# wreuven/h264-scroll-encoder

Measured on AMD Instinct MI355X. Metric: composed frames/sec (1280x720, 360x360 dyn) at 1/2/4/8 GPU; bit-exact vs CPU, higher is better.
Workload: dtype u8; 1 GPU; BASELINE config 3: 256 concurrent 1280x720 streams + 360x360 synthetic dynamic rect (4x4 int transform + quant + CAVLC), composer_write_scroll_frame semantics; resolution=1280x720, streams_per_gpu=256, parallelism=static stream shard x1, no RCCL

## Files before the change

h264-scroll-encoder_amd/csrc/dyn_device.h:

```cpp
#ifndef SCROLL_DYN_DEVICE_H
#define SCROLL_DYN_DEVICE_H

#include "qparams.h"
#include "scroll_device.h"

namespace scroll {
namespace dyn {

constexpr int QP_DEFAULT = 26, QP_MIN = 22, QP_MAX = 51, LEVEL_MAX = 2063;
__host__ __device__ constexpr int mf_of(int r, int cls)
{
    constexpr int T[6][3] = {{13107, 5243, 8066}, {11916, 4660, 7490}, {10082, 4194, 6554},
                             {9362, 3647, 5825},  {8192, 3355, 5243},  {7282, 2893, 4559}};
    return T[r][cls];
}
__host__ __device__ constexpr QParams qparams(int qp)
{
    return QParams{mf_of(qp % 6, 0), mf_of(qp % 6, 1), mf_of(qp % 6, 2), 15 + qp / 6, (1 << (15 + qp / 6)) / 6};
}
__device__ __host__ inline QParams qparams_rt(int qp)
{
    const int r = qp % 6, b = 15 + qp / 6;
    const int m0 = r == 0 ? 13107 : r == 1 ? 11916 : r == 2 ? 10082 : r == 3 ? 9362 : r == 4 ? 8192 : 7282;
    const int m1 = r == 0 ? 5243 : r == 1 ? 4660 : r == 2 ? 4194 : r == 3 ? 3647 : r == 4 ? 3355 : 2893;
// ... 881 lines not shown
        const int p = top_bit(mm);
        mm &= ~(1u << p);
        const int run = pprev - p - 1;
        const uint32_t e = P.rb[(zl < 7 ? zl : 7) - 1][run];
        push(acc, an, e & 255u, e >> 8, cap);
        zl -= run;
        pprev = p;
    }
    if constexpr (LB) {
        if (cap.n == 0) {
            cap.lo = acc;
            cap.n = an;
            ok = true;
            return tc;
        }
    }
    if (an > 32u) cap.put((uint32_t)(acc >> 32), (int)(an - 32u));
    cap.put((uint32_t)acc, an > 32u ? 32 : (int)an);
    ok = cap.n <= 128;
    return tc;
}

constexpr int TZRB_N = 65536 + 32768;
__device__ __host__ inline uint32_t tzrb_entry(const Tabs &T, uint32_t nz, int maxc)
{
    const int tc = __builtin_popcount(nz);
    if (tc == 0) return 1u << 31;
    uint32_t acc = 0;
    int n = 0;
    const int hi = 31 - __builtin_clz(nz), tz = hi + 1 - tc;
    if (tc < maxc) {
        acc = T.tz_bits[tc - 1][tz];
        n = T.tz_len[tc - 1][tz];
    }
    int zl = tz, p = hi;
    uint32_t m = nz & ~(1u << hi);
    for (int k = 1; k < tc && zl > 0; ++k) {
        const int q = 31 - __builtin_clz(m);
        m &= ~(1u << q);
        const int run = p - q - 1, zi = (zl < 7 ? zl : 7) - 1;
        acc = (acc << T.rb_len[zi][run]) | T.rb_bits[zi][run];
        n += T.rb_len[zi][run];
        zl -= run;
        p = q;
    }
    return (n ? acc << (32 - n) : 0u) | (1u << (31 - n));
}

constexpr int LVT_V = 47, LVT_W = 96, LVT_C = 9, LVT_N = LVT_C * LVT_W, LVT_ROW = 4 * LVT_W;
__device__ __host__ constexpr uint32_t lvt_entry(int c, int v)
{
    if (v == 0 || v > LVT_V || v < -LVT_V) return 0u;
    const int sl = c >= 7 ? c - 7 : c, adj = c >= 7 ? 2 : 0;
    const int a = v < 0 ? -v : v;
    const int code = 2 * a - 2 + (v < 0 ? 1 : 0) - adj;
    if (code < 0) return 0u;
    const int lim = sl ? (15 << sl) : 30;
    const uint32_t mk = (1u << sl) - 1u;
    uint32_t fv = ((uint32_t)code & mk) | (mk + 1u), fl = (uint32_t)((code >> sl) + 1 + sl);
    if (code >= lim) {
        fv = (uint32_t)(4096 + code - lim);
        fl = 28u;
    } else if (sl == 0 && code >= 14) {
        fv = (uint32_t)(code + 2);
        fl = 19u;
    }
    const int s1 = sl == 0 ? 1 : sl;
    const int nx = s1 + ((a > (3 << (s1 - 1)) && s1 < 6) ? 1 : 0);
    return fv | fl << 13 | (uint32_t)(nx * LVT_ROW) << 18;
}
struct LvTab {
    uint32_t e[LVT_N];
};
constexpr LvTab make_lvt()
{
    LvTab T{};
    for (int c = 0; c < LVT_C; ++c)
        for (int i = 0; i < LVT_W; ++i) T.e[c * LVT_W + i] = lvt_entry(c, i - LVT_V - 1);
    return T;
}

template <class CAP>
__device__ __host__ inline int cavlc_body_t(CAP &cap, const int8_t *lb, uint32_t nz, uint32_t tzrb, int &t1o,
                                            bool &ok, const uint32_t *lvt)
{
    const int tc = __builtin_popcount(nz);
    const uint32_t g0 = (nz << 1) | 1u;
    const int c0 = __builtin_clz(g0);
    const uint32_t g1 = g0 & ~((0x80000000u >> c0) & ~1u);
    const int c1 = __builtin_clz(g1);
    const uint32_t g2 = g1 & ~((0x80000000u >> c1) & ~1u);
    const int c2 = __builtin_clz(g2);
    const uint32_t g3 = g2 & ~((0x80000000u >> c2) & ~1u);
    const int v0 = lb[30 - c0], v1 = lb[30 - c1], v2 = lb[30 - c2];
    const bool o0 = c0 < 31 && v0 * v0 == 1, o1 = o0 && c1 < 31 && v1 * v1 == 1;
    const bool o2 = o1 && c2 < 31 && v2 * v2 == 1;
    const int t1 = (int)o0 + (int)o1 + (int)o2;
    t1o = t1;
    ok = true;
    if (tc == 0) return 0;
    const uint32_t s3 = ((uint32_t)v0 >> 31) << 2 | ((uint32_t)v1 >> 31) << 1 | ((uint32_t)v2 >> 31);
    uint64_t acc = s3 >> (3 - t1);
    uint32_t an = (uint32_t)t1;
    uint32_t g = t1 == 0 ? g0 : (t1 == 1 ? g1 : (t1 == 2 ? g2 : g3));
    uint32_t m = g >> 1;
    auto push = [](uint64_t &ac, uint32_t &n, uint32_t v, uint32_t len, CAP &c) {
        uint32_t n2 = n + len;
        if (n2 > 64u) {
            if (n > 32u) c.put((uint32_t)(ac >> 32), (int)(n - 32u));
            c.put((uint32_t)ac, n > 32u ? 32 : (int)n);
            ac = 0;
            n2 = len;
        }
        ac = (ac << len) | v;
        n = n2;
    };
    uint32_t cls = (uint32_t)((((tc > 10 && t1 < 3) ? 1 : 0) + (t1 < 3 ? 7 : 0)) * LVT_ROW);
    auto entry = [lvt](uint32_t row, int v) -> uint32_t {
        return *reinterpret_cast<const uint32_t *>(reinterpret_cast<const char *>(lvt + LVT_V + 1) + ((int)row + 4 * v));
    };
    auto level_code = [&](int v, uint32_t row) -> uint32_t {
        if (v >= -LVT_V && v <= LVT_V) return entry(row, v);
        const int cl = (int)row / LVT_ROW;
        const int sl = cl >= 7 ? cl - 7 : cl, adj = cl >= 7 ? 2 : 0;
        const int a = v < 0 ? -v : v;
        const int code = 2 * a - 2 + (v < 0 ? 1 : 0) - adj;
        const int lim = sl ? (15 << sl) : 30;
        const uint32_t mk = (1u << sl) - 1u;
        uint32_t fv = ((uint32_t)code & mk) | (mk + 1u);
        uint32_t fl = (uint32_t)((code >> sl) + 1 + sl);
        const bool e15 = code >= lim, e14 = sl == 0 && code >= 14;
        fv = e15 ? (uint32_t)(4096 + code - lim) : (e14 ? (uint32_t)(code + 2) : fv);
        fl = e15 ? 28u : (e14 ? 19u : fl);
        const int s1 = sl == 0 ? 1 : sl;
        return fv | fl << 13 | (uint32_t)((s1 + ((a > (3 << (s1 - 1)) && s1 < 6) ? 1 : 0)) * LVT_ROW) << 18;
    };
    const uint32_t m0 = m, an0 = an;
    const uint64_t acc0 = acc;
    const uint32_t cls0 = cls;
    const CAP cap0 = cap;
    uint32_t big = 0;
    int cn = __builtin_clz(g);
    int vn = (int)lb[30 - cn];
    while (g > 1u) {
        const int v = vn;
        g &= ~(0x80000000u >> cn);
        cn = __builtin_clz(g);
        vn = (int)lb[30 - cn];
        const int vc = v < -LVT_V ? -LVT_V : (v > LVT_V ? LVT_V : v);
        big |= (uint32_t)(vc ^ v);
        const uint32_t e = entry(cls, vc);
        push(acc, an, e & 0x1fffu, (e >> 13) & 31u, cap);
        cls = e >> 18;
    }
    if (big) {
        m = m0;
        an = an0;
        acc = acc0;
        cls = cls0;
        cap = cap0;
        for (int k = t1; k < tc; ++k) {
            const int p = top_bit(m);
            m &= ~(1u << p);
            const uint32_t e = level_code((int)lb[p], cls);
            push(acc, an, e & 0x1fffu, (e >> 13) & 31u, cap);
            cls = e >> 18;
        }
    }
    const uint32_t tzl = 31u - (uint32_t)__builtin_ctz(tzrb);
    push(acc, an, (tzrb >> 1) >> (31u - tzl), tzl, cap);
    if (cap.n == 0) {
        cap.lo = acc;
        cap.n = an;
        return tc;
    }
    if (an > 32u) cap.put((uint32_t)(acc >> 32), (int)(an - 32u));
    cap.put((uint32_t)acc, an > 32u ? 32 : (int)an);
    ok = cap.n <= 128;
    return tc;
}

template <class CAP, class PT>
__device__ __host__ inline int cavlc_dc4(CAP &cap, const PT &P, const int c[4])
{
    const uint32_t nz = (c[0] != 0 ? 1u : 0u) | (c[1] != 0 ? 2u : 0u) | (c[2] != 0 ? 4u : 0u) |
                        (c[3] != 0 ? 8u : 0u);
// ... 109 lines not shown
```

h264-scroll-encoder_amd/csrc/dyn_kernels.hip:

```cpp
#include <hip/hip_runtime.h>

#include <stdint.h>
#include <mutex>

#include "dyn_device.h"
#include "dyn_engine.h"
#include "nal_ctx.h"
#include "stage_util.h"

using namespace scroll;
using namespace scroll::dyn;
using namespace scroll::stage;

namespace {

__constant__ Tabs g_tabs = SCROLL_DYN_TABS;
constexpr Tabs k_tabs = SCROLL_DYN_TABS;
__constant__ PTabs g_ptabs = make_ptabs(k_tabs);
__device__ uint32_t g_tzrb[TZRB_N];
struct QpPair {
    QParams l, c;
};
struct QpTab {
    QpPair q[QP_MAX + 1];
// ... 904 lines not shown
                     rowstage + nb * g.rs_frame_words + rs_runs_words(g, nA, gi), EPC_STATIC - 1, t, GW);
        wave_sync();
    }
    if (t == 0) rowstage[nb * g.rs_frame_words + rs_runs_words(g, nA, gi)] = L.ncand;
}


__device__ inline CapSink cap_of_msb(uint64_t a, uint64_t b, uint32_t n)
{
    if (n == 0u) return CapSink{0, 0, 0};
    const uint32_t sh = 128u - n;
    if (sh >= 64u) return CapSink{0, a >> (sh - 64u), n};
    if (sh == 0u) return CapSink{a, b, n};
    return CapSink{a >> sh, (b >> sh) | (a << (64u - sh)), n};
}

__device__ inline void put_piece(uint32_t *buf, uint32_t p0, uint32_t n, uint32_t pos, uint32_t tv, uint32_t tl,
                                 uint4 b, uint32_t bl)
{
    const uint32_t tw = tv & low_mask((int)tl);
    const uint32_t c0 = __builtin_amdgcn_alignbit(tw, b.x, tl), c1 = __builtin_amdgcn_alignbit(b.x, b.y, tl);
    const uint32_t c2 = __builtin_amdgcn_alignbit(b.y, b.z, tl), c3 = __builtin_amdgcn_alignbit(b.z, b.w, tl);
    const uint32_t c4 = __builtin_amdgcn_alignbit(b.w, 0u, tl);
    const uint32_t sh = pos & 31u;
    const uint32_t o[6] = {c0 >> sh, __builtin_amdgcn_alignbit(c0, c1, sh), __builtin_amdgcn_alignbit(c1, c2, sh),
                           __builtin_amdgcn_alignbit(c2, c3, sh), __builtin_amdgcn_alignbit(c3, c4, sh),
                           __builtin_amdgcn_alignbit(c4, 0u, sh)};
    const uint32_t nw = (sh + tl + bl + 31u) >> 5, w0 = (pos >> 5) - p0;
#pragma unroll
    for (uint32_t j = 0; j < 6; ++j)
        if (j < nw && w0 + j < n && o[j]) atomicOr(&buf[w0 + j], o[j]);
}

constexpr uint32_t ROW_PAD = 4;

__device__ inline void put_piece1(uint32_t *buf, uint32_t pos, uint32_t tv, uint32_t tl, uint4 b, uint32_t bl)
{
    const uint32_t tw = tv & low_mask((int)tl);
    const uint32_t c0 = __builtin_amdgcn_alignbit(tw, b.x, tl), c1 = __builtin_amdgcn_alignbit(b.x, b.y, tl);
    const uint32_t c2 = __builtin_amdgcn_alignbit(b.y, b.z, tl), c3 = __builtin_amdgcn_alignbit(b.z, b.w, tl);
    const uint32_t c4 = __builtin_amdgcn_alignbit(b.w, 0u, tl);
    const uint32_t sh = pos & 31u, nw = (sh + tl + bl + 31u) >> 5;
    uint32_t *d = buf + (pos >> 5);
    atomicOr(d, c0 >> sh);
    if (nw > 1u) atomicOr(d + 1, __builtin_amdgcn_alignbit(c0, c1, sh));
    if (nw > 2u) atomicOr(d + 2, __builtin_amdgcn_alignbit(c1, c2, sh));
    if (nw > 3u) {
        atomicOr(d + 3, __builtin_amdgcn_alignbit(c2, c3, sh));
        if (nw > 4u) {
            atomicOr(d + 4, __builtin_amdgcn_alignbit(c3, c4, sh));
            if (nw > 5u) atomicOr(d + 5, __builtin_amdgcn_alignbit(c4, 0u, sh));
        }
    }
}

constexpr int ROW_MAXT = 1024;
#ifndef SCROLL_ROW_WAVES
#define SCROLL_ROW_WAVES 8
#endif
#ifndef SCROLL_ROW_NP
#define SCROLL_ROW_NP 3
#endif
#ifndef SCROLL_ROW_NP_WIDE
#define SCROLL_ROW_NP_WIDE 4
#endif
#ifndef SCROLL_ROW_WIDE
#define SCROLL_ROW_WIDE 40
#endif
constexpr int ROW_NPMAX = 8;
#ifndef SCROLL_ROW_GB
#define SCROLL_ROW_GB 896
#endif
constexpr int ROW_GB = SCROLL_ROW_GB;

constexpr int ROW_PCD_N = (NPC + 3) & ~3;

struct RowFixed {
    RowTabs ptabs;
    uint32_t pcd[ROW_PCD_N];
    union {
        uint32_t buf[ROW_GB + 4];
        struct {
            uint32_t kc[2][SORT_KEYS];
            uint32_t kc_pad[32 - 2 * SORT_KEYS];
            uint32_t lvt[LVT_N];
        };
    };
    uint64_t hhi[12], hlo[12];
    uint32_t hlen[12];
    int32_t wo[8], wl[8], wv[8];
    int32_t head_over;
    uint32_t rt[32];
    uint32_t ncand;
    uint32_t spill;
};

static_assert(2 * SORT_KEYS <= 32 && 32 + LVT_N <= ROW_GB, "the sort counts and the level table share the bit window");
static_assert(ROW_PAD == 4, "RowFixed::buf holds ROW_PAD spare words");
static_assert(sizeof(RowFixed) <= 4992, "eight config-3 row workgroups per CU");

__host__ __device__ inline size_t row_lds_base(int w)
{
    return (size_t)16 * NPC * w + (size_t)4 * (w + 1) + (size_t)2 * (3 * NPC * w) + (size_t)10 * w + 16;
}
#ifndef SCROLL_ROW_GB_WIDE
#define SCROLL_ROW_GB_WIDE 1248
#endif
constexpr int ROW_GB_WIDE = SCROLL_ROW_GB_WIDE;
__host__ __device__ inline size_t row_wide_off(int w) { return (row_lds_base(w) + 15) & ~(size_t)15; }
__host__ __device__ inline bool row_wide_win(int w)
{
    return w > SCROLL_ROW_WIDE && row_wide_off(w) + 4 * (size_t)(ROW_GB_WIDE + ROW_PAD) + sizeof(RowFixed) <= 163840;
}
__host__ __device__ inline size_t row_lds_bytes(int w)
{
    return row_wide_win(w) ? row_wide_off(w) + 4 * (size_t)(ROW_GB_WIDE + ROW_PAD) : row_lds_base(w);
}

__host__ __device__ constexpr uint32_t pc_desc(int pc)
{
    if (pc == 16 || pc == 17) return 1u << 17;
    int da = 0, db = 0, e = 0;
    bool al = false, bt = false;
    if (pc < 16) {
        const int bx = pc & 3, by = pc >> 2;
        al = bx == 0;
        da = al ? 3 - NPC : -1;
        bt = by == 0;
        db = bt ? 0 : -4;
        e = bt ? pc : 0;
    } else {
        const int b = (pc - 18) & 3, bx = b & 1, by = b >> 1;
        al = bx == 0;
        da = al ? 1 - NPC : -1;
        bt = by == 0;
        db = bt ? 0 : -2;
        e = bt ? (pc < 22 ? pc - 14 : pc - 16) : 0;
    }
    return (uint32_t)(da + 32) | (al ? 1u : 0u) << 6 | (uint32_t)(db + 32) << 7 | (bt ? 1u : 0u) << 13 |
           (uint32_t)e << 14;
}

struct alignas(16) RowConst {
    RowTabs ptabs;
    uint32_t pcd[ROW_PCD_N];
    uint32_t lvt[LVT_N];
};
constexpr RowConst make_rowconst(const Tabs &T)
{
    RowConst C{};
    const PTabs P = make_ptabs(T);
    for (int i = 0; i < 4 * 68; ++i) C.ptabs.ct[i / 68][i % 68] = P.ct[i / 68][i % 68];
    for (int i = 0; i < 12; ++i) C.ptabs.tzdc[i / 4][i % 4] = P.tzdc[i / 4][i % 4];
    for (int i = 0; i < 7 * 16; ++i) C.ptabs.rb[i / 16][i % 16] = P.rb[i / 16][i % 16];
    for (int i = 0; i < NPC; ++i) C.pcd[i] = pc_desc(i);
    const LvTab V = make_lvt();
    for (int i = 0; i < LVT_N; ++i) C.lvt[i] = V.e[i];
    return C;
}
__constant__ RowConst g_rowconst = make_rowconst(k_tabs);
constexpr int ROWC_NV = (int)(sizeof(RowConst) / 16), ROWC_HEAD = (int)(offsetof(RowConst, lvt) / 16);
constexpr int ROWC_GAP = (int)((offsetof(RowFixed, lvt) - offsetof(RowConst, lvt)) / 16);
static_assert(offsetof(RowFixed, ptabs) == 0 && offsetof(RowFixed, pcd) == offsetof(RowConst, pcd) &&
                  offsetof(RowFixed, kc) == offsetof(RowConst, lvt) && offsetof(RowFixed, lvt) % 16 == 0 &&
                  sizeof(RowConst) % 16 == 0 && sizeof(RowConst) == 16 * ROWC_HEAD + 4 * LVT_N,
              "RowConst is RowFixed's head without the sort's words");
static_assert(offsetof(RowFixed, wl) == offsetof(RowFixed, wo) + 32 && offsetof(RowFixed, wv) == offsetof(RowFixed, wo) + 64 &&
                  offsetof(PlanPending, wl) == offsetof(PlanPending, wo) + 32 &&
                  offsetof(PlanPending, wv) == offsetof(PlanPending, wo) + 64,
              "the waypoint table copies as 24 words");

struct EpfLds {
    uint32_t *goff, *gb, *gw, *cw, *cbase, *lst, *cnt;
    uint32_t *ws;
};
__host__ __device__ inline int row_chroma0(int w) { return (16 * w + 63) & ~63; }
__host__ __device__ inline int row_vtasks(int w) { return row_chroma0(w) + 8 * w; }

__host__ __device__ inline int row_threads(int w)
{
    const int nt = row_vtasks(w), np = w > SCROLL_ROW_WIDE ? SCROLL_ROW_NP_WIDE : SCROLL_ROW_NP;
    const int a = (((nt + np - 1) / np) + 63) & ~63;
    const int b = (((nt + ROW_NPMAX - 1) / ROW_NPMAX) + 63) & ~63;
    const int t = a > b ? a : b;
    return t < ROW_MAXT ? t : ROW_MAXT;
}

struct BlkPix {
    uint32_t a[4], b[4], c;
};

__device__ inline __amdgpu_buffer_rsrc_t buf_rsrc(const void *p, uint32_t n)
{
    return __builtin_amdgcn_make_buffer_rsrc(const_cast<void *>(p), (short)0, (int)n, 0x00020000);
}

struct FetchOff {
    uint32_t s, b[4], c;
    int pb;
};

__device__ inline void fetch_luma(FetchOff &o, int v, int ry, const DynGeom &g, const uint32_t *rt)
{
    const int k = v >> 4, r = v & 15, bx = r & 3, by = r >> 2;
    o.s = (uint32_t)((16 * ry + 4 * by) * (16 * g.w) + 16 * k + 4 * bx);
    const uint32_t po = (uint32_t)(16 * (g.x0 + k) + 4 * bx);
#pragma unroll
    for (int i = 0; i < 4; ++i) o.b[i] = po + rt[4 * by + i];
    o.c = o.b[3];
}

__device__ inline void fetch_chroma(FetchOff &o, int e, int ry, const DynGeom &g, uint32_t csz, const uint32_t *ru,
                                    const uint32_t *rd)
{
    const int ndt = g.w * g.h, k = e >> 3, p = (e >> 2) & 1, r = e & 3, bx = r & 1, by = r >> 1;
    o.s = (uint32_t)(256 * ndt + (p ? 64 * ndt : 0) + (8 * ry + 4 * by) * (8 * g.w) + 8 * k + 4 * bx);
    const uint32_t co = (uint32_t)p * csz + (uint32_t)(8 * (g.x0 + k) + 4 * bx);
#pragma unroll
    for (int i = 0; i < 4; ++i) o.b[i] = co + (ru[4 * by + i] & ROW_OFF);
    o.c = co + (rd[4 * by + 3] & ROW_OFF);
}

__device__ inline void fetch_pass9(const FetchOff &o, uint32_t adv, uint32_t stride, __amdgpu_buffer_rsrc_t fs,
                                   __amdgpu_buffer_rsrc_t rb, BlkPix &px)
{
#pragma unroll
    for (int i = 0; i < 4; ++i) {
        px.a[i] = __builtin_amdgcn_raw_buffer_load_b32(fs, o.s, adv + (uint32_t)i * stride, 0);
        px.b[i] = __builtin_amdgcn_raw_buffer_load_b32(rb, o.b[i], adv, 0);
    }
    px.c = __builtin_amdgcn_raw_buffer_load_b32(rb, o.c, adv, 0);
}

__device__ inline uint32_t bilin4(uint32_t b, uint32_t c, uint32_t f)
{
    const uint32_t g = 8u - f;
    const uint32_t be = b & 0x00ff00ffu, bo = (b >> 8) & 0x00ff00ffu;
    const uint32_t ce = c & 0x00ff00ffu, co = (c >> 8) & 0x00ff00ffu;
    const uint32_t ve = __umul24(g, be) + __umul24(f, ce) + 0x00040004u;
    const uint32_t vo = __umul24(g, bo) + __umul24(f, co) + 0x00040004u;
    return ((ve >> 3) & 0x00ff00ffu) | (((vo >> 3) & 0x00ff00ffu) << 8);
}

static_assert(NPC == 26 && NPC * DYN_MAX_W < 18724, "div_npc's reciprocal (10083 / 2^18) is exact below 18724");
__device__ inline int div_npc(int i) { return (int)(__umul24((uint32_t)i, 10083u) >> 18); }

__device__ inline int row_slot(int task, int w)
{
    const int jj = task - 16 * w;
    const bool l = jj < 0;
    const int k = l ? task >> 4 : jj >> 3, pc = l ? task & 15 : 18 + (jj & 7);
    return (int)__umul24((uint32_t)k, (uint32_t)NPC) + pc;
}

struct RowArgs {
    DevStream *st;
    const NalDesc *nal;
    const PlanPending *pend;
    DynFrame *dfr;
    const uint32_t *rows;
    const uint8_t *src, *refs;
    const uint4 *heads;
    int32_t ld_nal, ld_fr;
    DynGeom g;
    unsigned long long *tcx;
    uint32_t epoch, pad0;
    uint32_t *rowstage, *gbits, *spill, *ctr;
    const uint16_t *meta;
    const uint2 *blo, *bhi;
    const uint4 *bwd;
    uint64_t *stamps;
};
static_assert(std::is_trivially_copyable<RowArgs>::value && std::is_standard_layout<RowArgs>::value,
              "RowArgs is copied into the kernel-argument segment as it is: offsetof = kernarg offset");
static_assert(offsetof(RowArgs, st) == 0 && alignof(RowArgs) == 8 && sizeof(RowArgs) % 8 == 0,
              "the only kernel parameter starts the kernel-argument segment");
static_assert(offsetof(RowArgs, tcx) % 16 == 0 && offsetof(RowArgs, epoch) == offsetof(RowArgs, tcx) + 8,
              "tcx and epoch: one 16-byte scalar load");
static_assert(offsetof(RowArgs, gbits) == offsetof(RowArgs, rowstage) + 8 &&
                  offsetof(RowArgs, ctr) == offsetof(RowArgs, rowstage) + 24,
              "phase 5's four pointers are adjacent");

typedef const char __attribute__((address_space(4))) *KargPtr;
__device__ inline KargPtr kargs_here()
{
    KargPtr p = (KargPtr)__builtin_amdgcn_kernarg_segment_ptr();
    asm volatile("" : "+s"(p));
    return p;
}
template <class T>
__device__ inline T karg_at(KargPtr p, size_t off)
{
    return *reinterpret_cast<const T __attribute__((address_space(4))) *>(p + off);
}
#define row_arg(K, F) karg_at<decltype(RowArgs::F)>(K, offsetof(RowArgs, F))

__device__ inline void row_copy_tabs(RowFixed &L, int s, size_t nb, int lane)
{
    constexpr int NK = (ROWC_NV + 63) / 64;
    const KargPtr K = kargs_here();
    const int32_t *pw = reinterpret_cast<const int32_t *>(reinterpret_cast<const char *>(row_arg(K, pend) + s) +
                                                          offsetof(PlanPending, wo));
    const uint4 *hv = row_arg(K, heads) + nb * DYN_HEAD_VECS;
    const uint4 *src = reinterpret_cast<const uint4 *>(&g_rowconst);
    const int l24 = min(lane, 23), l12 = min(lane, 11);
    uint4 v[NK];
#pragma unroll
    for (int k = 0; k < NK; ++k) v[k] = src[min(lane + 64 * k, ROWC_NV - 1)];
    const int32_t wp = pw[l24];
    const uint4 m = hv[l12];
    const uint32_t hl = reinterpret_cast<const uint32_t *>(hv + 12)[l12];
    uint4 *dst = reinterpret_cast<uint4 *>(&L);
#pragma unroll
    for (int k = 0; k < NK; ++k) {
        const int i = min(lane + 64 * k, ROWC_NV - 1);
        dst[i + (i >= ROWC_HEAD ? ROWC_GAP : 0)] = v[k];
    }
    reinterpret_cast<int32_t *>(reinterpret_cast<char *>(&L) + offsetof(RowFixed, wo))[l24] = wp;
    L.hhi[l12] = (uint64_t)m.x << 32 | m.y;
    L.hlo[l12] = (uint64_t)m.z << 32 | m.w;
    L.hlen[l12] = hl & 0x7fffffffu;
    const bool over = __builtin_amdgcn_ballot_w64(lane < 12 && (hl >> 31)) != 0;
    if (lane == 0) L.head_over = over;
}

template <bool GEN, bool DBG>
__global__ __launch_bounds__(ROW_MAXT) __attribute__((amdgpu_waves_per_eu(SCROLL_ROW_WAVES))) void k_dyn_row(const RowArgs a)
{
    __shared__ RowFixed L;
    extern __shared__ uint4 rdyn[];
    const DynGeom &g = a.g;
    uint64_t *const stamps = DBG ? a.stamps : nullptr;
    const uint64_t t_entry = stamps ? __builtin_amdgcn_s_memrealtime() : 0ull;
    const int r = blockIdx.x, t = threadIdx.x, T = blockDim.x, lane = t & 63, wave = t >> 6, nwv = T >> 6;
    int f = blockIdx.y, s = blockIdx.z;
    const int ld_fr = a.ld_fr;
    if (GEN) {
        const uint32_t *ctr = a.ctr;
        const uint32_t j = blockIdx.y, n = min(__builtin_amdgcn_readfirstlane(ctr[1]), g.gen_cap);
        if (j >= n) return;
        const uint32_t q = __builtin_amdgcn_readfirstlane(ctr[DYN_CTR_LIST + j]);
        s = (int)(q / (uint32_t)ld_fr);
        f = (int)(q - (uint32_t)s * (uint32_t)ld_fr);
    }
    const size_t nb = (size_t)s * ld_fr + f;
    constexpr bool general = GEN;
    constexpr int SR = DYN_STATIC_ROWS;
    uint64_t *stp = nullptr;
    if (DBG && stamps) stp = stamps + (((size_t)s * gridDim.y + f) * g.ngroups + (max(1, (g.y0 + SR - 1) / SR) + r)) * 8;
    if (stp && t == 0) stp[0] = t_entry;
    const Rect R{g.x0, g.y0, g.w, g.h};
    const int w = R.w, ndt = R.w * R.h, row = R.y0 + r, npc = NPC * w, ntask = 24 * w;
    const int nA = max(1, (R.y0 + SR - 1) / SR);
    const DevStream *S = a.st + s;
    const uint32_t *const rows = a.rows;
    const int mbw = g.pw / 16;
    const uint32_t ysz = (uint32_t)g.pw * (uint32_t)g.ph, csz = ysz / 4;
    const int L0 = row_chroma0(w), nl = 16 * w, ntv = L0 + 8 * w;
    const int np = (ntv + T - 1) / T;
    const int wv0 = 64 * __builtin_amdgcn_readfirstlane(wave);
    auto kind_of = [&](int q) -> int {
        const int v0 = q * T + wv0;
        return v0 < nl ? 0 : (v0 < ntv ? 1 : 2);
    };
    const __amdgpu_buffer_rsrc_t fs = buf_rsrc(a.src + (size_t)s * g.src_ld + (size_t)f * g.src_fr, (uint32_t)g.src_fr);
    const __amdgpu_buffer_rsrc_t rb = buf_rsrc(a.refs + (size_t)s * g.ref_ld, 3u * ysz);
    const DynFrame df = a.dfr[nb];
    FetchOff fo;
    fo.pb = -1;
    bool fo_chroma = false;
    BlkPix nx;
    if (!general) {
        const uint32_t *rtg = rows + nb * (size_t)(32 * g.h);
        const int k0 = kind_of(0);
        const int e = t & 31;
        const uint32_t rtv = rtg[e < 16 ? 16 * r + e : 16 * g.h + (e < 24 ? 8 * r + e - 16 : 8 * g.h + 8 * r + e - 24)];
        if (k0 == 0) {
            fetch_luma(fo, t, r, g, rtg + 16 * r);
            fo.pb = 0;
            fetch_pass9(fo, 0u, (uint32_t)(16 * w), fs, rb, nx);
            nx.c = 0u;
            L.rt[e] = rtv;
        } else if (k0 == 1) {
            fetch_chroma(fo, t - L0, r, g, csz, rtg + 16 * g.h + 8 * r, rtg + 24 * g.h + 8 * r);
            fo.pb = 0;
            fo_chroma = true;
            fetch_pass9(fo, 0u, (uint32_t)(8 * w), fs, rb, nx);
        }
    }
    if (df.nal < 0 || ((df.err & DF_GENERAL) != 0) != GEN) return;

    uint4 *lv = rdyn;
    uint32_t *moff = reinterpret_cast<uint32_t *>(lv + npc);
    uint16_t *mt = reinterpret_cast<uint16_t *>(moff + w + 1), *lo = mt + npc, *off16 = lo + npc;
    uint16_t *order = off16;
    uint8_t *ta = reinterpret_cast<uint8_t *>(off16 + npc), *cbpa = ta + 8 * w, *codea = cbpa + w;
    uint32_t *mbits = reinterpret_cast<uint32_t *>(ta);

    if (t == 0) L.ncand = 0;
    if (t < SORT_KEYS) L.kc[0][t] = 0u;
    if (general && wv0 == T - 64) row_copy_tabs(L, s, nb, lane);
    const int qpy = __builtin_amdgcn_readfirstlane((int)df.ep);
    const QParams ql = g_qptab.q[qpy].l, qc = g_qptab.q[qpy].c;
    const HeadSel HS = head_sel(S, a.nal[(size_t)s * a.ld_nal + df.nal]);
    if (!general)
        asm volatile(""
                     :
                     : "s"(HS.a_end), "s"(HS.mbw), "s"(ql.mf0), "s"(ql.mf1), "s"(ql.mf2), "s"(ql.qbits), "s"(ql.qf),
                       "s"(qc.mf0), "s"(qc.mf1), "s"(qc.mf2), "s"(qc.qbits), "s"(qc.qf));

    __syncthreads();
    if (!general) {
        static_assert(ROW_MAXT % 64 == 0, "row_threads gives whole waves: the per-pass step T is a multiple of 64");
        const uint32_t frc = __builtin_amdgcn_readfirstlane((L.rt[16] >> 28) & 7u);
        const int qL = nl > wv0 ? (nl - wv0 + T - 1) / T : 0;
        const int qC = ntv > wv0 ? (ntv - wv0 + T - 1) / T : 0;
        auto issue_l = [&](int q, BlkPix &px) {
            fetch_pass9(fo, (uint32_t)((q - fo.pb) * T), (uint32_t)(16 * w), fs, rb, px);
        };
        auto issue_c = [&](int q, BlkPix &px) {
            if (!fo_chroma) {
                fetch_chroma(fo, q * T + t - L0, r, g, csz, L.rt + 16, L.rt + 24);
                fo.pb = q;
                fo_chroma = true;
            }
            fetch_pass9(fo, (uint32_t)((q - fo.pb) * T), (uint32_t)(8 * w), fs, rb, px);
        };
        auto issue_any = [&](int q, BlkPix &px) {
            if (q < qL) issue_l(q, px);
            else issue_c(q, px);
        };
        const NzConst nzc = nz_const();
        auto put_rec = [&](int slot, const uint32_t pk[4]) {
            const uint4 p4 = make_uint4(pk[0], pk[1], pk[2], pk[3]);
            const uint32_t nz = nz_mask16_c(p4, nzc);
            const int n = __builtin_popcount(nz);
            lv[slot] = p4;
            mt[slot] = (uint16_t)nz;
            if (n) lo[slot] = (uint16_t)atomicAdd(&L.kc[0][SORT_KEYS - 1 - min(n, SORT_KEYS - 1)], 1u);
        };
        const LevelsBias bl = levels_bias(ql), bc = levels_bias(qc);
        auto code_l = [&](int q, const BlkPix &px) {
            const int v = q * T + t;
            uint32_t pk[4];
            int w0 = 0;
            levels_pk<true>(px.a, px.b, pk, w0, ql, bl.k1, bl.k0);
            if (v < nl) put_rec((int)__umul24((uint32_t)(v >> 4), (uint32_t)NPC) + (v & 15), pk);
        };
        auto code_c = [&](int q, const BlkPix &px) {
            const int e = q * T + t - L0;
            uint32_t pr[4], pk[4];
            int w0 = 0;
            if (frc == 4u) {
#pragma unroll
                for (int i = 0; i < 4; ++i) pr[i] = __builtin_amdgcn_lerp(px.b[i], i < 3 ? px.b[i + 1] : px.c, 0x01010101u);
            } else if (frc == 0u) {
#pragma unroll
                for (int i = 0; i < 4; ++i) pr[i] = px.b[i];
            } else {
#pragma unroll
                for (int i = 0; i < 4; ++i) pr[i] = bilin4(px.b[i], i < 3 ? px.b[i + 1] : px.c, frc);
            }
            levels_pk<false>(px.a, pr, pk, w0, qc, bc.k1, bc.k0);
            const bool ok = e < 8 * w;
            if (ok) put_rec((int)__umul24((uint32_t)(e >> 3), (uint32_t)NPC) + 18 + (e & 7), pk);
            if (ok) reinterpret_cast<int16_t *>(lv + (e >> 3) * NPC + 16 + ((e >> 2) & 1))[e & 3] = (int16_t)w0;
        };
        BlkPix A = nx, B;
        int q = 0;
        for (; q + 1 < qL; q += 2) {
            issue_l(q + 1, B);
            code_l(q, A);
            issue_any(q + 2, A);
            code_l(q + 1, B);
        }
        if (q < qL) {
            issue_any(q + 1, B);
            code_l(q, A);
            A = B;
            ++q;
        }
        for (; q + 1 < qC; q += 2) {
            issue_c(q + 1, B);
            code_c(q, A);
            issue_c(q + 2, A);
            code_c(q + 1, B);
        }
        if (q < qC) code_c(q, A);
        if (wv0 == T - 64) row_copy_tabs(L, s, nb, lane);
        __syncthreads();
        if (stp && t == 0) stp[1] = __builtin_amdgcn_s_memrealtime();
        const bool nopub = DBG && (g.debug & SCROLL_DEBUG_DYN_NOPUBLISH) && s == 0 && f == 0 && r == 0;
        if (t < w && r + 1 < R.h && !nopub) {
            const KargPtr K = kargs_here();
            unsigned long long *const tcx = row_arg(K, tcx);
            const uint32_t epoch = row_arg(K, epoch);
            const uint16_t *mk = mt + t * NPC;
            uint64_t v = 0;
#pragma unroll
            for (int e = 0; e < 8; ++e) {
                const int pcA = e < 4 ? 12 + e : (e < 6 ? 16 + e : 18 + e);
                v |= (uint64_t)__builtin_popcount(mk[pcA]) << (5 * e);
            }
            lb_store(tcx + (nb * R.h + r) * (size_t)w + t, (uint64_t)(epoch & 0xffffffu) << 40 | v);
        }
        {
            const uint32_t tot = lane < SORT_KEYS ? L.kc[0][lane] : 0u;
            uint32_t kb = tot;
            kb += dpp_or0<0x111, 0xf>(kb);
            kb += dpp_or0<0x112, 0xf>(kb);
            kb += dpp_or0<0x114, 0xf>(kb);
            kb += dpp_or0<0x118, 0xf>(kb);
            if (lane < SORT_KEYS) L.kc[1][lane] = kb - tot;
            wave_sync();
        }
        for (int task = t; task < ntask; task += T) {
            const int slot = row_slot(task, w);
            const int tcs = __builtin_popcount(mt[slot]);
            if (tcs) {
                order[L.kc[1][SORT_KEYS - 1 - min(tcs, SORT_KEYS - 1)] + lo[slot]] =
                    (uint16_t)(slot | (task < 16 * w ? 0 : 0x8000));
            }
        }
        __syncthreads();
        const int zbase = (int)L.kc[1][SORT_KEYS - 1];
        for (int pa = 0; pa < np; ++pa) {
            const int pos = pa * T + t;
            if (pos >= zbase) continue;
            const uint32_t oe = order[pos];
            const int slot = (int)(oe & 0x7fffu);
            const bool luma = !(oe & 0x8000u);
            CapSink cap{0, 0, 0};
            int t1 = 0;
            bool ok = true;
            const uint32_t nz = mt[slot];
            const uint32_t tzrb = g_tzrb[luma ? nz : 65536u + nz];
            const int tc = cavlc_body_t(cap, reinterpret_cast<const int8_t *>(lv + slot), nz, tzrb, t1, ok, L.lvt);
            mt[slot] = ok ? (uint16_t)(cap.n | (uint32_t)tc << 8 | (uint32_t)t1 << 13)
                          : (uint16_t)((uint32_t)tc << 8 | (uint32_t)t1 << 13 | M_OVF);
            if (ok) lv[slot] = body_msb(cap.hi, cap.lo, cap.n);
        }
        const int dcT = nwv > 1 ? T - 64 : T;
        for (int i = dcT - 1 - t; i >= 0 && i < 2 * w; i += dcT) {
            const int k = i >> 1, p = i & 1, sl = k * NPC + 16 + p;
            const uint4 q = lv[sl];
            const int d0 = (int)(int16_t)(q.x & 0xffffu), d1 = (int)(int16_t)(q.x >> 16);
            const int d2 = (int)(int16_t)(q.y & 0xffffu), d3 = (int)(int16_t)(q.y >> 16);
            const int dq[4] = {quant_dc(d0 + d1 + d2 + d3, qc), quant_dc(d0 - d1 + d2 - d3, qc),
                               quant_dc(d0 + d1 - d2 - d3, qc), quant_dc(d0 - d1 - d2 + d3, qc)};
            CapSink cap{0, 0, 0};
            const int tc = cavlc_dc4(cap, L.ptabs, dq);
            if (cap.n <= 128) {
                mt[sl] = (uint16_t)(cap.n | (uint32_t)tc << 8);
                lv[sl] = body_msb(cap.hi, cap.lo, cap.n);
            } else {
                mt[sl] = (uint16_t)((uint32_t)tc << 8 | M_OVF);
                lv[sl] = make_uint4(((uint32_t)dq[0] & 0xffffu) | (uint32_t)dq[1] << 16,
                                    ((uint32_t)dq[2] & 0xffffu) | (uint32_t)dq[3] << 16, 0u, 0u);
            }
        }
    } else {
        const int q0 = r * w;
        const size_t gs = df.rbsp_bytes;
        const uint16_t *M = a.meta + gs * (size_t)(NPC * ndt);
        const uint2 *BL = a.blo + gs * (size_t)(NPC * ndt), *BH = a.bhi + gs * (size_t)(NPC * ndt);
        for (int i = t; i < npc; i += T) {
            const int k = div_npc(i), pc = i - k * NPC;
            const int rec = rec_of(q0 + k, pc, ndt);
            const uint16_t mv = M[rec];
            mt[i] = mv;
            uint4 bv = make_uint4(0u, 0u, 0u, 0u);
            if ((mv & 255u) || (mv & M_OVF)) {
                const uint4 bd = get_body(BL, BH, rec, (mv & 255u) > 64u || (mv & M_OVF));
                bv = (mv & M_OVF) ? bd
                                  : body_msb((uint64_t)bd.z | (uint64_t)bd.w << 32,
                                             (uint64_t)bd.x | (uint64_t)bd.y << 32, mv & 255u);
            }
            lv[i] = bv;
        }
        for (int i = t; i < 8 * w; i += T) {
            const int k = i >> 3, e = i & 7;
            const int pcA = e < 4 ? 12 + e : (e < 6 ? 16 + e : 18 + e);
            ta[i] = r > 0 ? (uint8_t)tc_of(M[rec_of(q0 + k - w, pcA, ndt)]) : (uint8_t)0;
        }
    }
    if (!general && wave == nwv - 1) {
        const KargPtr K = kargs_here();
        const unsigned long long *const tcx = row_arg(K, tcx);
        const uint32_t epoch = row_arg(K, epoch);
        uint64_t prev = r > 0 ? __builtin_amdgcn_s_memrealtime() : 0ull, waited = 0;
        bool late = false;
        for (int k = lane; k < w; k += 64) {
            uint64_t v = 0;
            if (r > 0) {
                const unsigned long long *p = tcx + (nb * R.h + r - 1) * (size_t)w + k;
                for (;;) {
                    v = __hip_atomic_load(p, __ATOMIC_RELAXED, __HIP_MEMORY_SCOPE_AGENT);
                    if ((uint32_t)(v >> 40) == (epoch & 0xffffffu)) break;
                    const uint64_t now = __builtin_amdgcn_s_memrealtime(), gap = now - prev;
                    prev = now;
                    if (gap < HANDOFF_GAP) waited += gap;
                    if (waited > HANDOFF_TICKS) {
                        v = 0;
                        late = true;
                        break;
                    }
                    __builtin_amdgcn_s_sleep(1);
                }
            }
#pragma unroll
            for (int e = 0; e < 8; ++e) ta[8 * k + e] = (uint8_t)((v >> (5 * e)) & 31u);
        }
        if (__builtin_amdgcn_ballot_w64(late) != 0 && lane == 0) atomicOr(&row_arg(K, dfr)[nb].err, DF_HANDOFF);
    }
    const bool wide = GEN && __builtin_amdgcn_readfirstlane((int)df.ep) < QP_MIN;
    auto ovf_wide = [&](int k, int pc) -> const uint4 * {
        if (!wide) return nullptr;
        return a.bwd + (size_t)df.rbsp_bytes * (size_t)(NPC * ndt) + rec_of(r * w + k, pc, ndt);
    };
    __syncthreads();
    if (stp && t == 0) stp[2] = __builtin_amdgcn_s_memrealtime();

    const Tabs &TB = g_tabs;
    const PTabs &PT = *reinterpret_cast<const PTabs *>(&g_ptabs);
    const uint16_t(*ctab)[68] = L.ptabs.ct;
    const int nAe = R.x0 > 0 ? 0 : -1, nBe = row > 0 ? 0 : -1;
    auto token = [&](int i, int k, int pc, uint32_t D) {
        const uint32_t mv = mt[i];
        const int ia = max(i + (int)(D & 63u) - 32, 0), ib = max(i + (int)((D >> 7) & 63u) - 32, 0);
        const int tA = tc_of(mt[ia]), tB = tc_of(mt[ib]), tT = (int)ta[8 * k + (int)((D >> 14) & 7u)];
        const int nA = ((D & 64u) && k == 0) ? nAe : tA;
        const int nB = (D & 8192u) ? (r > 0 ? tT : nBe) : tB;
        const int mean = (nA + nB + 1) >> 1, one = max(max(nA, nB), 0);
        const int nC0 = (nA | nB) >= 0 ? mean : one;
        const int nC = (D >> 17) ? -1 : nC0;
        const int tc = tc_of(mv), t1 = (int)((mv >> 13) & 3u);
        const uint32_t ce = ctab[nC < 0 ? 3 : (nC < 2 ? 0 : (nC < 4 ? 1 : 2))][4 * tc + t1];
        const uint32_t tl = nC < 0 ? 0u : (nC >= 8 ? 6u : ce >> 8);
        uint32_t len = tl + (mv & 255u);
        if (mv & M_OVF) len = ovf_bits(PT, TB, lv[i], ovf_wide(k, pc), pc, nC);
        uint32_t nc1 = (uint32_t)(nC + 1);
        if (!(mv & M_OVF) && nC >= 0 && len <= 128u) {
            const uint32_t tv = nC >= 8 ? (tc ? (uint32_t)(((tc - 1) << 2) | t1) : 3u) : (ce & 255u);
            const uint32_t tw = tv & low_mask((int)tl);
            const uint4 b = lv[i];
            lv[i] = make_uint4(__builtin_amdgcn_alignbit(tw, b.x, tl), __builtin_amdgcn_alignbit(b.x, b.y, tl),
                               __builtin_amdgcn_alignbit(b.y, b.z, tl), __builtin_amdgcn_alignbit(b.z, b.w, tl));
            mt[i] = (uint16_t)((mv & ~255u) | len);
            nc1 = 0u;
        }
        lo[i] = (uint16_t)(len | nc1 << 11);
    };
    const uint32_t cbtab = TB.cbp_code[min(lane, 47)];
    for (int i = t; i < npc; i += T) {
        const int k = div_npc(i), pc = i - k * NPC;
        token(i, k, pc, L.pcd[pc]);
    }
    __syncthreads();
    if (stp && t == 0) stp[3] = __builtin_amdgcn_s_memrealtime();
    const bool head_over = L.head_over;
    auto head_slow = [&]() -> HeadCtx {
        const KargPtr K = kargs_here();
        const int nalj = row_arg(K, dfr)[nb].nal;
        const NalDesc d = row_arg(K, nal)[(size_t)s * row_arg(K, ld_nal) + nalj];
        return head_ctx(nal_ctx(row_arg(K, st) + s, d, L.wo, L.wl, L.wv));
    };
    auto head_bits = [&](int rr, int col) -> uint32_t {
        if (!head_over) return L.hlen[HS.sel(rr, col)];
        CountSink cn{0};
        head_slow().put_slow(cn, rr, col);
        return cn.n;
    };

    {
        const int j = t & 7, G = T >> 3;
        const bool lum = j < 4, four = j != 4;
        const int pb = lum ? 8 * (j >> 1) + 2 * (j & 1) : (j == 4 ? 16 : (j == 5 ? 18 : 22));
        const int d2 = lum ? 4 : 2, d3 = d2 + 1;
        for (int k0 = wv0 >> 3; k0 < w; k0 += G) {
            const int k = k0 + (lane >> 3);
            const bool live = k < w && j < 7;
            const int i0 = (int)__umul24((uint32_t)k, (uint32_t)NPC) + pb;
            uint32_t mm = 0u, l0 = 0u, l1 = 0u, l2 = 0u, l3 = 0u;
            if (live) {
                mm = (uint32_t)mt[i0] | mt[i0 + 1];
                l0 = lo[i0] & LO_LEN;
                l1 = lo[i0 + 1] & LO_LEN;
                if (four) {
                    mm |= (uint32_t)mt[i0 + d2] | mt[i0 + d3];
                    l2 = lo[i0 + d2] & LO_LEN;
                    l3 = lo[i0 + d3] & LO_LEN;
                }
            }
            const uint64_t nzw = __builtin_amdgcn_ballot_w64((mm & 0x1f00u) != 0u);
            const uint32_t m = (uint32_t)(nzw >> (lane & 56)) & 0x7fu;
            const uint32_t cbp_l = m & 15u, cbp_c = (m & 0x60u) ? 2u : (m >> 4);
            const uint32_t cbp = cbp_l | cbp_c << 4;
            const uint32_t code = (uint32_t)__shfl((int)cbtab, (int)cbp, 64);
            const bool pres = lum ? (m >> j) & 1u : (j == 4 ? cbp_c >= 1u : cbp_c == 2u);
            const uint32_t tot = pres ? l0 + l1 + l2 + l3 : 0u;
            uint32_t incl = tot, u;
            u = dpp_or0<0x111, 0xf>(incl);
            incl += j >= 1 ? u : 0u;
            u = dpp_or0<0x112, 0xf>(incl);
            incl += j >= 2 ? u : 0u;
            u = dpp_or0<0x114, 0xf>(incl);
            incl += j >= 4 ? u : 0u;
            const uint32_t hb = head_bits(row, R.x0 + min(k, w - 1)) + ue_bits(code) + (cbp ? 1u : 0u);
            const uint32_t o0 = hb + incl - tot, no = pres ? 0u : 0xffffu;
            if (live) {
                off16[i0] = (uint16_t)(o0 | no);
                off16[i0 + 1] = (uint16_t)((o0 + l0) | no);
                if (four) {
                    off16[i0 + d2] = (uint16_t)((o0 + l0 + l1) | no);
                    off16[i0 + d3] = (uint16_t)((o0 + l0 + l1 + l2) | no);
                }
            }
            if (j == 7 && k < w) {
                mbits[k] = hb + incl;
                cbpa[k] = (uint8_t)cbp;
                codea[k] = (uint8_t)code;
            }
        }
    }
    const int x1 = R.x0 + w;
    const uint32_t h0 = head_bits(row, 0) + 1u;
    const uint32_t h1 = mbw >= 3 ? head_bits(row, 1) + 1u : 0u;
    const uint32_t h2 = mbw >= 2 ? head_bits(row, mbw - 1) + 1u : 0u;
    auto colpos = [&](int col) -> uint32_t {
        if (col <= R.x0) return col == 0 ? 0u : h0 + (uint32_t)(col - 1) * h1;
        if (col < x1) return moff[col - R.x0];
        return moff[w] + (uint32_t)(col - x1) * h1 + (col == mbw && x1 <= mbw - 1 ? h2 - h1 : 0u);
    };
    __syncthreads();
    const int gi = nA + r;
    const uint32_t mb0 = R.x0 == 0 ? 0u : h0 + (uint32_t)(R.x0 - 1) * h1;
    if (w <= 64) {
        const uint32_t len = lane < w ? mbits[lane] : 0u;
        const uint32_t incl = wave_incl_sum_dpp(len);
// ... 30 lines not shown
    bool lost = false;
    if (((bits + 31u) >> 5) > epc) {
        const KargPtr K = kargs_here();
        const uint32_t rs_spill_words = row_arg(K, g.rs_spill_words);
        if (t == 0) L.spill = atomicAdd(&row_arg(K, ctr)[0], 1u);
        __syncthreads();
        const uint32_t k = L.spill;
        uint32_t *fr = rowstage + nb * rs_frame_words;
        uint32_t *sp = row_arg(K, spill) + (size_t)k * rs_spill_words;
        if (k >= row_arg(K, g.rs_spill_cap) || (uint64_t)(sp - fr) + rs_spill_words > 0x3fffffffull) {
            if (t == 0) atomicOr(&row_arg(K, dfr)[nb].err, DF_OVER);
            lost = true;
        } else {
            if (t == 0) out[epc] = 0x80000000u | (uint32_t)(sp - fr);
            out = sp;
            epc = rs_spill_words - EPC_ROW;
        }
    }
    const uint32_t nw = lost ? 0u : min((bits + 31u) >> 5, epc);
    const int npass = (int)((nw + GBW - 1) / GBW);
    for (int pi = 0; pi < npass; ++pi) {
        const uint32_t p0 = (uint32_t)pi * GBW;
        const uint32_t n = min((uint32_t)GBW, nw - p0);
        for (uint32_t i = (uint32_t)t; i < n; i += (uint32_t)T) wb[i] = 0u;
        __syncthreads();
        const LdsOrWin win{wb, p0, n};
        const bool one = npass == 1;
        for (int col = t; col < mbw; col += T) {
            const uint32_t pos = colpos(col);
            if (!one && (pos >= 32u * (p0 + n) || colpos(col + 1) <= 32u * p0)) continue;
            const int k = col - R.x0;
            const bool in = k >= 0 && k < w;
            if (one && !head_over) {
                const int cls = HS.sel(row, col);
                const uint32_t hl = L.hlen[cls];
                uint32_t tv = 1u, tn = 1u;
                if (in) {
                    const uint32_t x = (uint32_t)codea[k] + 1u, lz = 31u - (uint32_t)__builtin_clz(x);
                    tv = x;
                    tn = 2u * lz + 1u;
                    if (cbpa[k]) {
                        tv = tv << 1 | 1u;
                        ++tn;
                    }
                }
                if (hl + tn <= 128u) {
                    const uint64_t ha = L.hhi[cls], hb = L.hlo[cls];
                    const uint32_t t32 = tv << (32u - tn), q = hl >> 5, r = hl & 31u;
                    uint32_t wv[4] = {(uint32_t)(ha >> 32), (uint32_t)ha, (uint32_t)(hb >> 32), (uint32_t)hb};
#pragma unroll
                    for (uint32_t j = 0; j < 4; ++j)
                        wv[j] |= (j == q ? t32 >> r : 0u) | (j == q + 1u && r ? t32 << (32u - r) : 0u);
                    put_piece1(wb, pos, 0u, 0u, make_uint4(wv[0], wv[1], wv[2], wv[3]), hl + tn);
                    continue;
                }
            }
            WSink sk{win, 0, 0, 0};
            sk.start(pos);
            if (!head_over) {
                const int cls = HS.sel(row, col);
                sk.put_cap(cap_of_msb(L.hhi[cls], L.hlo[cls], L.hlen[cls]));
            } else {
                head_slow().put_slow(sk, row, col);
            }
            if (!in) {
                sk.put(1, 1);
            } else {
                put_ue(sk, (uint32_t)codea[k]);
                if (cbpa[k]) put_se(sk, 0);
            }
            sk.finish();
        }
        for (int i = t; i < npc; i += T) {
            const uint32_t o = off16[i];
            if (o == 0xffffu) continue;
            const int k = div_npc(i), pc = i - k * NPC;
            const uint32_t e = lo[i], mv = mt[i];
            const uint32_t pos = moff[k] + o;
            if (!one && (pos >= 32u * (p0 + n) || pos + (e & LO_LEN) <= 32u * p0)) continue;
            const int nC = (int)(e >> 11) - 1;
            const uint4 bd = lv[i];
            if (!(mv & M_OVF)) {
                if (nC == -1) {
                    if (one) put_piece1(wb, pos, 0u, 0u, bd, mv & 255u);
                    else put_piece(wb, p0, n, pos, 0u, 0u, bd, mv & 255u);
                } else {
                    uint32_t tv = 0, tl = 0;
                    piece_token(ctab, mv, nC, tv, tl);
                    if (one) put_piece1(wb, pos, tv, tl, bd, mv & 255u);
                    else put_piece(wb, p0, n, pos, tv, tl, bd, mv & 255u);
                }
            } else {
                ovf_put((LdsWords)wb, p0, n, pos, PT, TB, bd, ovf_wide(k, pc), pc, nC);
            }
        }
        __syncthreads();
        flush_window(wb, n, p0, p0 + n >= nw, out, &L.ncand, out + epc, EPC_ROW - 1, t, T);
        __syncthreads();
    }
    if (t == 0 && !lost) out[epc] = L.ncand;
    if (stp && t == 0) {
        stp[5] = __builtin_amdgcn_s_memrealtime();
        stp[6] = bits;
        stp[7] = (uint64_t)(uint32_t)__builtin_amdgcn_s_getreg((31 << 11) | 4);
    }
}

#ifndef SCROLL_EPS_KW
#define SCROLL_EPS_KW 4
#endif
constexpr int EPS_KW = SCROLL_EPS_KW;
static_assert(EPS_KW % 4 == 0, "the EP scan reads 16-byte LDS vectors");
__host__ __device__ inline size_t gtab_bytes(int ng, bool epfix)
{
    return (size_t)4 * (epfix ? 5 * (size_t)ng + 2 : 3 * (size_t)ng + 1);
}
struct GTab {
    uint32_t *goff, *gb, *gw, *cw, *cbase;
};
__device__ inline GTab gtab_of(uint32_t *p, int ng)
{
    GTab T;
    T.goff = p;
    T.gb = p + ng + 1;
    T.gw = T.gb + ng;
    T.cw = T.gw + ng;
    T.cbase = T.cw + ng;
    return T;
}

__device__ inline uint32_t rs_word_span(uint32_t P, int &gg, int ng, uint32_t T, const uint32_t *goff,
                                       const uint32_t *gb, const uint32_t *gw, const uint32_t *fr)
{
    uint32_t acc = 0, filled = 0;
    while (filled < 32u && gg < ng && P + filled < T) {
        const uint32_t lp = P + filled - goff[gg];
        if (lp >= gb[gg]) {
            ++gg;
            continue;
        }
        const uint32_t take = min(32u - filled, gb[gg] - lp);
        const uint32_t *src = fr + gw[gg];
        const uint32_t i = lp >> 5, sh = lp & 31u;
        uint32_t x = src[i];
        if (sh) {
            x <<= sh;
            if (32u - sh < take) x |= src[i + 1] >> (32u - sh);
        }
        x &= take >= 32u ? 0xffffffffu : ~(0xffffffffu >> take);
        acc |= x >> filled;
        filled += take;
    }
    return acc;
}

__device__ inline int rs_group_at(uint32_t P, int ng, const uint32_t *goff)
{
    int lo = 0, hi = ng;
    while (hi - lo > 1) {
        const int mid = (lo + hi) >> 1;
        if (goff[mid] <= P) lo = mid;
        else hi = mid;
    }
    return lo;
}

struct ScanLoads {
    uint32_t x0[EPS_KW], x1[EPS_KW], y[EPS_KW];
// ... 1427 lines not shown
```

Before: 3.197 million frames/s.

## Fold coeff_token into CAVLC body encoding for inner luma blocks in row kernel

Computes nC for each inner block during the sort pass and passes it to cavlc_body_t, which now emits the coeff_token together with the trailing-ones and level bits. Zero-coefficient inner blocks get their token written directly. The later token pass then only handles the edge blocks (8 per macroblock), plus an overflow fix-up loop that runs only when a shared ovf flag is set. This removes a separate per-block token pass over most blocks, in exchange for extra neighbour popcount work in the sort loop and more complex overflow bookkeeping that bit-exactness depends on.

```diff
diff --git a/h264-scroll-encoder_amd/csrc/dyn_device.h b/h264-scroll-encoder_amd/csrc/dyn_device.h
--- a/h264-scroll-encoder_amd/csrc/dyn_device.h
+++ b/h264-scroll-encoder_amd/csrc/dyn_device.h
@@ -987,7 +987,8 @@
 
 template <class CAP>
 __device__ __host__ inline int cavlc_body_t(CAP &cap, const int8_t *lb, uint32_t nz, uint32_t tzrb, int &t1o,
-                                            bool &ok, const uint32_t *lvt)
+                                            bool &ok, const uint32_t *lvt, int nC = -1,
+                                            const uint16_t (*ct)[68] = nullptr)
 {
     const int tc = __builtin_popcount(nz);
     const uint32_t g0 = (nz << 1) | 1u;
@@ -1003,10 +1004,22 @@
     const int t1 = (int)o0 + (int)o1 + (int)o2;
     t1o = t1;
     ok = true;
-    if (tc == 0) return 0;
+    uint32_t tv = 0u, tl = 0u;
+    if (nC >= 0) {
+        const uint32_t ce = ct[nC < 2 ? 0 : (nC < 4 ? 1 : 2)][4 * tc + t1];
+        tv = nC >= 8 ? (tc ? (uint32_t)(((tc - 1) << 2) | t1) : 3u) : (ce & 255u);
+        tl = nC >= 8 ? 6u : ce >> 8;
+    }
+    if (tc == 0) {
+        if (nC >= 0) {
+            cap.lo = tv;
+            cap.n = tl;
+        }
+        return 0;
+    }
     const uint32_t s3 = ((uint32_t)v0 >> 31) << 2 | ((uint32_t)v1 >> 31) << 1 | ((uint32_t)v2 >> 31);
-    uint64_t acc = s3 >> (3 - t1);
-    uint32_t an = (uint32_t)t1;
+    uint64_t acc = (uint64_t)(tv << t1 | s3 >> (3 - t1));
+    uint32_t an = tl + (uint32_t)t1;
     uint32_t g = t1 == 0 ? g0 : (t1 == 1 ? g1 : (t1 == 2 ? g2 : g3));
     uint32_t m = g >> 1;
     auto push = [](uint64_t &ac, uint32_t &n, uint32_t v, uint32_t len, CAP &c) {
diff --git a/h264-scroll-encoder_amd/csrc/dyn_kernels.hip b/h264-scroll-encoder_amd/csrc/dyn_kernels.hip
--- a/h264-scroll-encoder_amd/csrc/dyn_kernels.hip
+++ b/h264-scroll-encoder_amd/csrc/dyn_kernels.hip
@@ -1010,7 +1010,8 @@
         uint32_t buf[ROW_GB + 4];
         struct {
             uint32_t kc[2][SORT_KEYS];
-            uint32_t kc_pad[32 - 2 * SORT_KEYS];
+            uint32_t ovf;
+            uint32_t kc_pad[31 - 2 * SORT_KEYS];
             uint32_t lvt[LVT_N];
         };
     };
@@ -1023,7 +1024,7 @@
     uint32_t spill;
 };
 
-static_assert(2 * SORT_KEYS <= 32 && 32 + LVT_N <= ROW_GB, "the sort counts and the level table share the bit window");
+static_assert(2 * SORT_KEYS < 31 && 32 + LVT_N <= ROW_GB, "the sort counts, ovf and the level table share the bit window");
 static_assert(ROW_PAD == 4, "RowFixed::buf holds ROW_PAD spare words");
 static_assert(sizeof(RowFixed) <= 4992, "eight config-3 row workgroups per CU");
 
@@ -1172,14 +1173,6 @@
 
 static_assert(NPC == 26 && NPC * DYN_MAX_W < 18724, "div_npc's reciprocal (10083 / 2^18) is exact below 18724");
 __device__ inline int div_npc(int i) { return (int)(__umul24((uint32_t)i, 10083u) >> 18); }
-
-__device__ inline int row_slot(int task, int w)
-{
-    const int jj = task - 16 * w;
-    const bool l = jj < 0;
-    const int k = l ? task >> 4 : jj >> 3, pc = l ? task & 15 : 18 + (jj & 7);
-    return (int)__umul24((uint32_t)k, (uint32_t)NPC) + pc;
-}
 
 struct RowArgs {
     DevStream *st;
@@ -1326,6 +1319,7 @@
     uint32_t *mbits = reinterpret_cast<uint32_t *>(ta);
 
     if (t == 0) L.ncand = 0;
+    if (t == 0) L.ovf = 0u;
     if (t < SORT_KEYS) L.kc[0][t] = 0u;
     if (general && wv0 == T - 64) row_copy_tabs(L, s, nb, lane);
     const int qpy = __builtin_amdgcn_readfirstlane((int)df.ep);
@@ -1442,12 +1436,27 @@
             if (lane < SORT_KEYS) L.kc[1][lane] = kb - tot;
             wave_sync();
         }
+        const int nAs = g.x0 > 0 ? 0 : -1;
         for (int task = t; task < ntask; task += T) {
-            const int slot = row_slot(task, w);
+            const int jj = task - 16 * w;
+            const bool l = jj < 0;
+            const int k = l ? task >> 4 : jj >> 3, pc = l ? task & 15 : 18 + (jj & 7);
+            const int slot = (int)__umul24((uint32_t)k, (uint32_t)NPC) + pc;
+            const uint32_t D = L.pcd[pc];
             const int tcs = __builtin_popcount(mt[slot]);
+            const int ia = max(slot + (int)(D & 63u) - 32, 0), ib = slot + (int)((D >> 7) & 63u) - 32;
+            const int nB = __builtin_popcount(mt[ib]);
+            const int nA = ((D & 64u) && k == 0) ? (nAs < 0 ? nB : 0) : __builtin_popcount(mt[ia]);
+            const int nC = (nA + nB + 1) >> 1;
+            const bool inner = !(D & 8192u);
             if (tcs) {
-                order[L.kc[1][SORT_KEYS - 1 - min(tcs, SORT_KEYS - 1)] + lo[slot]] =
-                    (uint16_t)(slot | (task < 16 * w ? 0 : 0x8000));
+                order[L.kc[1][SORT_KEYS - 1 - min(tcs, SORT_KEYS - 1)] + lo[slot]] = (uint16_t)(slot | (l ? 0 : 0x8000));
+                lo[slot] = (uint16_t)(inner ? (uint32_t)(nC + 1) << 11 : 0u);
+            } else if (inner) {
+                const uint32_t ce = L.ptabs.ct[nC < 2 ? 0 : (nC < 4 ? 1 : 2)][0];
+                const uint32_t tl = nC >= 8 ? 6u : ce >> 8, tv = nC >= 8 ? 3u : (ce & 255u);
+                reinterpret_cast<uint32_t *>(lv + slot)[0] = tv << (32u - tl);
+                lo[slot] = (uint16_t)tl;
             }
         }
         __syncthreads();
@@ -1463,10 +1472,28 @@
             bool ok = true;
             const uint32_t nz = mt[slot];
             const uint32_t tzrb = g_tzrb[luma ? nz : 65536u + nz];
-            const int tc = cavlc_body_t(cap, reinterpret_cast<const int8_t *>(lv + slot), nz, tzrb, t1, ok, L.lvt);
-            mt[slot] = ok ? (uint16_t)(cap.n | (uint32_t)tc << 8 | (uint32_t)t1 << 13)
-                          : (uint16_t)((uint32_t)tc << 8 | (uint32_t)t1 << 13 | M_OVF);
-            if (ok) lv[slot] = body_msb(cap.hi, cap.lo, cap.n);
+            const int nC = (int)(lo[slot] >> 11) - 1;
+            const int tc = cavlc_body_t(cap, reinterpret_cast<const int8_t *>(lv + slot), nz, tzrb, t1, ok, L.lvt, nC,
+                                        L.ptabs.ct);
+            const uint32_t tm = (uint32_t)tc << 8 | (uint32_t)t1 << 13;
+            if (ok) {
+                mt[slot] = (uint16_t)(cap.n | tm);
+                lo[slot] = (uint16_t)cap.n;
+                lv[slot] = body_msb(cap.hi, cap.lo, cap.n);
+            } else {
+                uint32_t tv = 0, tl = 0;
+                if (nC >= 0) piece_token(L.ptabs.ct, tm, nC, tv, tl);
+                const uint32_t bn = cap.n - tl;
+                if (bn <= 128u) {
+                    mt[slot] = (uint16_t)(bn | tm);
+                    lo[slot] = (uint16_t)(cap.n | (uint32_t)(nC + 1) << 11);
+                    lv[slot] = body_msb(cap.hi, cap.lo, bn);
+                } else {
+                    mt[slot] = (uint16_t)(tm | M_OVF);
+                    lo[slot] = (uint16_t)((uint32_t)(nC + 1) << 11);
+                    L.ovf = 1u;
+                }
+            }
         }
         const int dcT = nwv > 1 ? T - 64 : T;
         for (int i = dcT - 1 - t; i >= 0 && i < 2 * w; i += dcT) {
@@ -1480,9 +1507,12 @@
             const int tc = cavlc_dc4(cap, L.ptabs, dq);
             if (cap.n <= 128) {
                 mt[sl] = (uint16_t)(cap.n | (uint32_t)tc << 8);
+                lo[sl] = (uint16_t)cap.n;
                 lv[sl] = body_msb(cap.hi, cap.lo, cap.n);
             } else {
                 mt[sl] = (uint16_t)((uint32_t)tc << 8 | M_OVF);
+                lo[sl] = 0u;
+                L.ovf = 1u;
                 lv[sl] = make_uint4(((uint32_t)dq[0] & 0xffffu) | (uint32_t)dq[1] << 16,
                                     ((uint32_t)dq[2] & 0xffffu) | (uint32_t)dq[3] << 16, 0u, 0u);
             }
@@ -1580,9 +1610,24 @@
         lo[i] = (uint16_t)(len | nc1 << 11);
     };
     const uint32_t cbtab = TB.cbp_code[min(lane, 47)];
-    for (int i = t; i < npc; i += T) {
-        const int k = div_npc(i), pc = i - k * NPC;
-        token(i, k, pc, L.pcd[pc]);
+    if constexpr (GEN) {
+        for (int i = t; i < npc; i += T) {
+            const int k = div_npc(i), pc = i - k * NPC;
+            token(i, k, pc, L.pcd[pc]);
+        }
+    } else {
+        if (L.ovf) {
+            for (int i = t; i < npc; i += T) {
+                const int k = div_npc(i), pc = i - k * NPC;
+                if (!(mt[i] & M_OVF) || (L.pcd[pc] & 8192u)) continue;
+                const uint32_t nc1 = (uint32_t)lo[i] >> 11;
+                lo[i] = (uint16_t)(ovf_bits(PT, TB, lv[i], nullptr, pc, (int)nc1 - 1) | nc1 << 11);
+            }
+        }
+        for (int i = t; i < 8 * w; i += T) {
+            const int k = i >> 3, j = i & 7, pc = j < 4 ? j : (j < 6 ? 14 + j : 16 + j);
+            token((int)__umul24((uint32_t)k, (uint32_t)NPC) + pc, k, pc, L.pcd[pc]);
+        }
     }
     __syncthreads();
     if (stp && t == 0) stp[3] = __builtin_amdgcn_s_memrealtime();
@@ -1779,8 +1824,8 @@
             const uint4 bd = lv[i];
             if (!(mv & M_OVF)) {
                 if (nC == -1) {
-                    if (one) put_piece1(wb, pos, 0u, 0u, bd, mv & 255u);
-                    else put_piece(wb, p0, n, pos, 0u, 0u, bd, mv & 255u);
+                    if (one) put_piece1(wb, pos, 0u, 0u, bd, e & LO_LEN);
+                    else put_piece(wb, p0, n, pos, 0u, 0u, bd, e & LO_LEN);
                 } else {
                     uint32_t tv = 0, tl = 0;
                     piece_token(ctab, mv, nC, tv, tl);
```

Result: faster. 3.237 million frames/s (median of 6 runs) (+1.2%).
